# EthanD11/RS-VIO

Hardware: AMD Instinct MI355X
Metric: stereo frames/sec (tracker+BA) on 752×480 EuRoC stream; BA ms/iter at window=10 (higher is better)
Workload: dtype f32 (tracker) / f64 (BA)

## Files before the change

### rs-vio_amd/csrc/ba.hip

```cpp
#include <rccl/rccl.h>

#include <algorithm>
#include <chrono>
#include <cmath>
#include <cstdlib>
#include <cstring>
#include <string>
#include <sys/resource.h>
#include <numeric>
#include <stdexcept>
#include <vector>

#include "common.hpp"

#include "obs_pass.hpp"
#include "se3.hpp"
#include "wave.hpp"

#pragma clang fp contract(fast)

namespace rsvio {

namespace {

// ... 351 lines not shown
            int u = 0;
#pragma unroll
            for (int a = 0; a < 3; ++a) {
#pragma unroll
                for (int c = 0; c < 3; ++c) L.Wr[a * 3 + c] += wt * (J[0][6 + a] * J[0][c] + J[1][6 + a] * J[1][c]);
#pragma unroll
                for (int c = a; c < 3; ++c) L.Ur[u++] += wt * (J[0][6 + a] * J[0][6 + c] + J[1][6 + a] * J[1][6 + c]);
                L.gr[a] += J[0][6 + a] * wr0 + J[1][6 + a] * wr1;
            }
        }
    }
}

__device__ __forceinline__ void wave_sync() {
    __builtin_amdgcn_fence(__ATOMIC_SEQ_CST, "wavefront");
    __builtin_amdgcn_wave_barrier();
}

template <bool WAVE = false>
__device__ void store_linearization(const Work& Wk, int buf, int s, int lane, bool act, bool fr, int first, int nk,
                                    int l, const SlotLin& L, double (*sh)[64]) {
    if (act && fr) {
        double rec[kRawF];
#pragma unroll
        for (int i = 0; i < 6; ++i) rec[RV + i] = L.V[i];
#pragma unroll
        for (int i = 0; i < 3; ++i) rec[RGP + i] = L.gp[i];
#pragma unroll
        for (int i = 0; i < 9; ++i) rec[RWR + i] = L.Wr[i];
#pragma unroll
        for (int i = 0; i < 6; ++i) rec[RUR + i] = L.Ur[i];
#pragma unroll
        for (int i = 0; i < 3; ++i) rec[RGR + i] = L.gr[i];
        rec[27] = 0.0;
        double2* dst = reinterpret_cast<double2*>(Wk.raws[buf] + (size_t)s * kRawF);
#pragma unroll
        for (int i = 0; i < kRawF / 2; ++i) dst[i] = make_double2(rec[2 * i], rec[2 * i + 1]);
    }
#pragma unroll
    for (int i = 0; i < 6; ++i) sh[i][lane] = L.V[i];
#pragma unroll
    for (int i = 0; i < 3; ++i) sh[6 + i][lane] = L.gp[i];
    if constexpr (WAVE) wave_sync(); else __syncthreads();
    if (act && lane == first) {
        double Vl[6] = {0, 0, 0, 0, 0, 0}, gl[3] = {0, 0, 0};
        for (int k = 0; k < nk; ++k) {
#pragma unroll
            for (int i = 0; i < 6; ++i) Vl[i] += sh[i][first + k];
#pragma unroll
            for (int i = 0; i < 3; ++i) gl[i] += sh[6 + i][first + k];
        }
        double rec[kLmF] = {Vl[0], Vl[1], Vl[2], Vl[3], Vl[4], Vl[5], gl[0], gl[1], gl[2], 0.0, 0.0, 0.0};
        double2* dst = reinterpret_cast<double2*>(Wk.rawl[buf] + (size_t)l * kLmF);
#pragma unroll
        for (int i = 0; i < kLmF / 2; ++i) dst[i] = make_double2(rec[2 * i], rec[2 * i + 1]);
    }
}

__device__ __forceinline__ bool chol_inv3(const double A[3][3], double X[3][3]) {
    const double d0 = A[0][0];
    if (!(d0 > 0.0) || !isfinite(d0)) return false;
    const double l00 = sqrt(d0), l10 = A[1][0] / l00, l20 = A[2][0] / l00;
    const double d1 = A[1][1] - l10 * l10;
    if (!(d1 > 0.0) || !isfinite(d1)) return false;
    const double l11 = sqrt(d1), l21 = (A[2][1] - l20 * l10) / l11;
    const double d2 = (A[2][2] - l20 * l20) - l21 * l21;
    if (!(d2 > 0.0) || !isfinite(d2)) return false;
    const double l22 = sqrt(d2);
    const double m00 = 1.0 / l00, m11 = 1.0 / l11, m22 = 1.0 / l22;
    const double m10 = -(l10 * m00) * m11, m21 = -(l21 * m11) * m22;
    const double m20 = -(l20 * m00 + l21 * m10) * m22;
    X[0][0] = (m00 * m00 + m10 * m10) + m20 * m20;
    X[0][1] = X[1][0] = m10 * m11 + m20 * m21;
    X[0][2] = X[2][0] = m20 * m22;
    X[1][1] = m11 * m11 + m21 * m21;
    X[1][2] = X[2][1] = m21 * m22;
    X[2][2] = m22 * m22;
    return true;
}

__device__ __forceinline__ bool landmark_inverse(const double* Vp, double lambda, double Vi[3][3], int chol) {
    double A[3][3] = {{Vp[0] + lambda, Vp[1], Vp[2]}, {Vp[1], Vp[3] + lambda, Vp[4]}, {Vp[2], Vp[4], Vp[5] + lambda}};
    const bool ok = chol ? chol_inv3(A, Vi) : inv3(A, Vi);
    if (!ok)
#pragma unroll
        for (int a = 0; a < 3; ++a)
#pragma unroll
            for (int c = 0; c < 3; ++c) Vi[a][c] = 0.0;
    return ok;
}

struct SlotSrc {
    const unsigned long long* mask;
    const int* lm_base;
    const int* wave_fill;
    const int* wave_lm;
    const unsigned* key;
    const double2* uv;
    int nb_lm, nb_pad;
    int uv32;
};
constexpr unsigned long long kEvenBits = 0x5555555555555555ull;

__device__ void build_slots_body(const Geometry& G, const Prob& Pr, const SlotSrc& S, int4* hdr, double2* huv,
                                 int b) {
    const int t = threadIdx.x;
    const double2 z2 = make_double2(0.0, 0.0);
    if (b < S.nb_lm) {
        const int l = 256 * b + t;
        if (l >= G.n_lm) return;
        const int base = S.lm_base[l];
        if (base < 0) return;
        const unsigned long long m = S.mask[l];
        unsigned long long kb = (m | (m >> 1)) & kEvenBits;
        const int ns = __popcll(kb);
        for (size_t ps = (size_t)base; kb; kb &= kb - 1, ++ps) {
            const int k = (__ffsll((long long)kb) - 1) >> 1;
            const int c0 = (int)(m >> (2 * k)) & 1, c1 = (int)(m >> (2 * k + 1)) & 1;
            const int no = c0 + c1;
            hdr[2 * ps] = make_int4(k, l, base & 63, ns);
            hdr[2 * ps + 1] = make_int4(Pr.free_idx[k], no, no == 2 ? 2 : c1, 0);
            if (no == 1) huv[2 * ps + 1] = z2;
        }
    } else if (b < S.nb_lm + S.nb_pad) {
        const int ps = 256 * (b - S.nb_lm) + t;
        if (ps >= 64 * G.n_wave || (ps & 63) < S.wave_fill[ps >> 6]) return;
        hdr[2 * (size_t)ps] = make_int4(0, 0, 0, 0);
        hdr[2 * (size_t)ps + 1] = make_int4(-1, 0, 0, 0);
        huv[2 * (size_t)ps] = z2;
        huv[2 * (size_t)ps + 1] = z2;
    } else {
        const int i = 256 * (b - S.nb_lm - S.nb_pad) + t;
        if (i >= G.n_obs) return;
        const unsigned key = S.key[i];
        const int l = (int)(key >> 6), k = (int)(key >> 1) & 31, c = (int)(key & 1);
        const unsigned long long m = S.mask[l];
        const unsigned long long below = ((m | (m >> 1)) & kEvenBits) & ((1ull << (2 * k)) - 1ull);
        const size_t q = (size_t)S.lm_base[l] + __popcll(below);
        const int sub = (c == 1 && ((m >> (2 * k)) & 1)) ? 1 : 0;
        if (S.uv32) {
            const float2 f = reinterpret_cast<const float2*>(S.uv)[i];
            huv[2 * q + sub] = make_double2((double)f.x, (double)f.y);
        } else {
            huv[2 * q + sub] = S.uv[i];
        }
    }
}

constexpr int kPairU = 8;

__device__ void build_pairs_body(const Geometry& G, const Prob& Pr, const SlotSrc& S, int4* pairs, int c) {
    __shared__ int cnt[4];
    const int pb = c / kGrp, x = c % kGrp;
    const int fa = Pr.pb_fa[pb], fb = Pr.pb_fb[pb];
    int kfa = 0, kfb = 0;
    for (int k = 0; k < G.n_kf; ++k) {
        const int f = Pr.free_idx[k];
        if (f == fa) kfa = k;
        if (f == fb) kfb = k;
    }
    const unsigned long long ma = 3ull << (2 * kfa), mb = 3ull << (2 * kfb);
    const unsigned long long below_a = (1ull << (2 * kfa)) - 1ull, below_b = (1ull << (2 * kfb)) - 1ull;
    const int tid = threadIdx.x, lane = tid & 63, wave = tid >> 6;
    const int nw = G.n_wave > x ? (G.n_wave - x + kGrp - 1) / kGrp : 0;
    const int k0 = nw * wave / 4, k1 = nw * (wave + 1) / 4;
    int4* out = pairs + (size_t)c * G.pair_stride;
    struct Round {
        int l0[kPairU], l1[kPairU], lbs[kPairU];
        unsigned long long m[kPairU];
    };
    auto load = [&](int kb, Round& R) {
#pragma unroll
        for (int u = 0; u < kPairU; ++u) {
            const int w = x + kGrp * (kb + u);
            const bool in = kb + u < k1;
            R.l0[u] = in ? S.wave_lm[w] : 0;
            R.l1[u] = in ? S.wave_lm[w + 1] : 0;
        }
#pragma unroll
        for (int u = 0; u < kPairU; ++u) {
            const bool in = R.l0[u] + lane < R.l1[u];
            R.m[u] = in ? S.mask[R.l0[u] + lane] : 0ull;
            R.lbs[u] = in ? S.lm_base[R.l0[u] + lane] : 0;
        }
    };
    auto scan = [&](const Round& R, bool write, int& acc) {
#pragma unroll
        for (int u = 0; u < kPairU; ++u) {
            for (int l = R.l0[u] + lane; l - lane < R.l1[u]; l += 64) {
                const bool first = l == R.l0[u] + lane;
                const unsigned long long mm = first ? R.m[u] : (l < R.l1[u] ? S.mask[l] : 0ull);
                const bool has = (mm & ma) && (mm & mb);
                const unsigned long long bal = __ballot(has);
                if (write && has) {
                    const unsigned long long kbits = (mm | (mm >> 1)) & kEvenBits;
                    const int lb = first ? R.lbs[u] : S.lm_base[l];
                    out[acc + __popcll(bal & ((1ull << lane) - 1ull))] =
                        make_int4(lb + __popcll(kbits & below_a), lb + __popcll(kbits & below_b), l, 0);
                }
                acc += __popcll(bal);
            }
        }
    };
    Round R0;
    load(k0, R0);
    int n = 0;
    scan(R0, false, n);
    for (int kb = k0 + kPairU; kb < k1; kb += kPairU) {
        Round R;
        load(kb, R);
        scan(R, false, n);
    }
    if (lane == 0) cnt[wave] = n;
    __syncthreads();
    int base = 0;
    for (int v = 0; v < wave; ++v) base += cnt[v];
    const int total = cnt[0] + cnt[1] + cnt[2] + cnt[3];
    scan(R0, true, base);
    for (int kb = k0 + kPairU; kb < k1; kb += kPairU) {
        Round R;
        load(kb, R);
        scan(R, true, base);
    }
    for (int i = total + tid; i < G.pair_stride; i += 256) out[i] = make_int4(-1, 0, 0, 0);
}

__global__ __launch_bounds__(256) void ba_stage_in(const uint4* src, uint4* __restrict__ dst, int n_words) {
    const int t = (int)(blockIdx.x * 256 + threadIdx.x), st = (int)(gridDim.x * 256);
    const int i0 = t, i1 = t + st;
    uint4 a, b;
    host_load2x16(src + min(i0, n_words - 1), src + min(i1, n_words - 1), a, b);
    if (i0 < n_words) dst[i0] = a;
    if (i1 < n_words) dst[i1] = b;
}

__global__ __launch_bounds__(256) void ba_build_layout(Geometry G, Prob Pr, SlotSrc S, int nb_slots, int4* hdr,
                                                       double2* huv, int4* pairs) {
    const int b = blockIdx.x;
    if (b < nb_slots)
        build_slots_body(G, Pr, S, hdr, huv, b);
    else
        build_pairs_body(G, Pr, S, pairs, b - nb_slots);
}

__device__ void linearize_body(const Geometry& G, const Prob& Pr, const Work& Wk, int w, int with_reset,
                               double lambda0) {
    __shared__ double sh[10][64];
    const int lane = threadIdx.x;
    const int s = 64 * w + lane;
    if (with_reset) {
        const int nt = G.n_wave * 64;
        for (int i = s; i < 7 * G.n_kf; i += nt) {
            Wk.pose[0][i] = Wk.pose_init[i];
            Wk.pose[1][i] = Wk.pose_init[i];
        }
        for (int i = s; i < 3 * G.n_lm; i += nt) {
            Wk.pw[0][i] = Wk.pw_init[i];
            Wk.pw[1][i] = Wk.pw_init[i];
        }
        if (s == 0) {
            Wk.tick[1] = wall_clock64();
            *Wk.singular = 0;
            LmState st{};
            st.lambda = lambda0;
            st.nu = 2.0;
            *Wk.st = st;
        }
    }
    const double* pose0 = with_reset ? Wk.pose_init : Wk.pose[0];
    const double* pw0 = with_reset ? Wk.pw_init : Wk.pw[0];
    const int4 h0 = Pr.slot_hdr[2 * s], h1 = Pr.slot_hdr[2 * s + 1];
    const double2 uvq[2] = {Pr.slot_uv[2 * s], Pr.slot_uv[2 * s + 1]};
    STAMP(11);
    const bool act = h1.y > 0;
    const int kf = h0.x, l = h0.y, first = act ? h0.z : lane, nk = act ? h0.w : 1;
    const bool fr = h1.x >= 0;
    SlotLin L;
    if (act) {
        const Pose P = pose_from7(pose0 + 7 * kf);
        const double* pwp = pw0 + 3 * l;
        const double p[3] = {pwp[0], pwp[1], pwp[2]};
        slot_linearize(G, P, p, h1.y, h1.z, uvq, fr, L);
    } else {
        const Pose P{};
        const double p[3] = {0.0, 0.0, 1.0};
        slot_linearize(G, P, p, 0, 0, uvq, false, L);
    }
    STAMP(12);
    store_linearization(Wk, 0, s, lane, act, fr, first, nk, l, L, sh);
    const double c = wave_sum_det(L.cost);
    if (lane == 0) {
        Wk.partA[w * kPartA] = c;
        Wk.partA[w * kPartA + 1] = 0.0;
    }
    STAMP(14);
}

__global__ __launch_bounds__(64) void ba_linearize(Geometry G, Prob Pr, Work Wk, double lambda0) {
    linearize_body(G, Pr, Wk, blockIdx.x, 1, lambda0);
}

__device__ void trial_scalars_wave(const Geometry& G, const Prob& Pr, const Work& Wk, const LmState& s,
                                   int include_poses, double out[4]) {
    const int lane = threadIdx.x & 63;
    constexpr int kU = 8;
    double4 pv[kU];
    const int wl = max(G.n_wave - 1, 0), el = 7 * G.n_kf - 1;
#pragma unroll
    for (int k = 0; k < kU; ++k)
        pv[k] = *reinterpret_cast<const double4*>(Wk.partD + (size_t)min(lane + 64 * k, wl) * kPartD);
    double p0[3], p1[3];
    int fi[3];
#pragma unroll
    for (int k = 0; k < 3; ++k) {
        const int e = min(lane + 64 * k, el);
        fi[k] = Pr.free_idx[e / 7];
        p0[k] = Wk.pose[0][e];
        p1[k] = Wk.pose[1][e];
    }
#pragma unroll
    for (int k = 0; k < kU; ++k)
        if (lane + 64 * k >= G.n_wave) pv[k] = make_double4(0.0, 0.0, 0.0, 0.0);
    bool fr[3];
#pragma unroll
    for (int k = 0; k < 3; ++k) fr[k] = include_poses && lane + 64 * k <= el && fi[k] >= 0;
    double acc[kPartD] = {0.0, 0.0, 0.0, 0.0};
#pragma unroll
    for (int k = 0; k < kU; ++k) {
        acc[0] += pv[k].x;
        acc[1] += pv[k].y;
        acc[2] += pv[k].z;
        acc[3] += pv[k].w;
    }
    for (int i = lane + 64 * kU; i < G.n_wave; i += 64) {
        const double4 v = *reinterpret_cast<const double4*>(Wk.partD + (size_t)i * kPartD);
        acc[0] += v.x;
        acc[1] += v.y;
        acc[2] += v.z;
        acc[3] += v.w;
    }
    double sq[2] = {0.0, 0.0};
#pragma unroll
    for (int k = 0; k < 3; ++k)
        if (fr[k]) {
            sq[0] += p0[k] * p0[k];
            sq[1] += p1[k] * p1[k];
        }
    if (!s.solve_ok)
#pragma unroll
        for (int k = 0; k < kPartD; ++k) acc[k] = 0.0;
    acc[3] += sq[s.cur];
#pragma unroll
    for (int k = 0; k < kPartD; ++k) out[k] = wave_sum_det(acc[k]);
}

__device__ void trial_scalars_p2p(const Geometry& G, const Prob& Pr, const Work& Wk, const LmState& s, const P2P& P,
                                  unsigned long long gen, int* err, double out[4]) {
    const int lane = threadIdx.x & 63, par = (int)(gen & 1);
    double* own = P.peer[P.rank];
    const int el = 7 * G.n_kf - 1;
    double p0[3], p1[3];
    int fi[3];
#pragma unroll
    for (int k = 0; k < 3; ++k) {
        const int e = min(lane + 64 * k, el);
        fi[k] = Pr.free_idx[e / 7];
        p0[k] = Wk.pose[0][e];
        p1[k] = Wk.pose[1][e];
    }
    double sq[2] = {0.0, 0.0};
#pragma unroll
    for (int k = 0; k < 3; ++k)
        if (lane + 64 * k <= el && fi[k] >= 0) {
            sq[0] += p0[k] * p0[k];
            sq[1] += p1[k] * p1[k];
        }
    for (int j = 0; j < 4; ++j) out[j] = 0.0;
    bool late = false;
    for (int r = 0; r < P.nranks; ++r) {
        const int nw = P.xnw[r];
        double acc[kPartD] = {0.0, 0.0, 0.0, 0.0};
        for (int w = lane; w < max(nw, 512); w += 64) {
            double4 v = make_double4(0.0, 0.0, 0.0, 0.0);
            if (w < nw) {
                const unsigned long long* f = p2p_tflag(own, par, r, w);
                long long spins = 0;
                while (__hip_atomic_load(f, __ATOMIC_RELAXED, __HIP_MEMORY_SCOPE_SYSTEM) < gen) {
                    __builtin_amdgcn_s_sleep(1);
                    if (++spins > (1ll << 25)) {
                        late = true;
                        break;
                    }
                }
                __builtin_amdgcn_fence(__ATOMIC_ACQUIRE, "");
                const double* q = p2p_tval(own, par, r, w);
// ... 2205 lines not shown
    for (int k = 1; k < kPartD; ++k) mv = i == k ? out[k] : mv;
    double got = mv;
    if (r < nr && r != me) {
        ll_put(p2p_ll(P.peer[r], par, me) + 2 * i, mv, g32);
        const unsigned long long* w = p2p_ll(P.peer[me], par, r) + 2 * i;
        long long spins = 0;
        for (;;) {
            const unsigned long long a = __hip_atomic_load(w, __ATOMIC_RELAXED, __HIP_MEMORY_SCOPE_SYSTEM);
            const unsigned long long b = __hip_atomic_load(w + 1, __ATOMIC_RELAXED, __HIP_MEMORY_SCOPE_SYSTEM);
            if ((unsigned)(a >> 32) == g32 && (unsigned)(b >> 32) == g32) {
                got = __longlong_as_double((long long)((a & 0xffffffffull) | (b << 32)));
                break;
            }
            if (++spins > (1ll << 25)) {
                late = true;
                got = 0.0;
                break;
            }
            __builtin_amdgcn_s_sleep(1);
        }
    }
    if (late) atomicExch(err, 1);
    double v4[kPartD];
#pragma unroll
    for (int k = 0; k < kPartD; ++k) {
        double v = 0.0;
        for (int q = 0; q < nr; ++q) v += rl64(got, 4 * q + k);
        v4[k] = v;
    }
    if (lane == 0) {
#pragma unroll
        for (int k = 0; k < kPartD; ++k) Wk.trial4[k] = v4[k];
        *xgen = gen;
    }
}

__global__ __launch_bounds__(64) void ba_backsub_relinearize_p2p3(Geometry G, Prob Pr, Work Wk, P2P P,
                                                                  unsigned long long* xgen, int* err,
                                                                  unsigned long long* k6tag) {
    __shared__ double sh[10][64];
    __shared__ double shp[3][64];
    __shared__ double shs[4][64];
    if ((int)blockIdx.x == G.n_wave) {
        if (G.n_wave <= 256)
            k6_reduce_p2p<4>(G, Pr, Wk, P, xgen, err, k6tag);
        else
            k6_reduce_p2p<8>(G, Pr, Wk, P, xgen, err, k6tag);
        return;
    }
    unsigned long long gen = *xgen + 1;
    __asm__ volatile("" : "+s"(gen));
    k6_body<false>(G, Pr, Wk, blockIdx.x, threadIdx.x, sh, shp, shs, nullptr, gen, k6tag);
}

__device__ void k6_last_push(const Geometry& G, const Prob& Pr, const Work& Wk, const P2P& P,
                             unsigned long long* xgen, unsigned long long gen, const unsigned long long* k6part,
                             const LmState& s) {
    const int lane = threadIdx.x & 63;
    constexpr int kU = 8;
    const int wl = max(G.n_wave - 1, 0), el = 7 * G.n_kf - 1;
    unsigned long long pw[kU][kPartD];
#pragma unroll
    for (int k = 0; k < kU; ++k)
#pragma unroll
        for (int j = 0; j < kPartD; ++j)
            pw[k][j] = __hip_atomic_load(k6part + (size_t)min(lane + 64 * k, wl) * kPartD + j, __ATOMIC_RELAXED,
                                         __HIP_MEMORY_SCOPE_AGENT);
    double p0[3], p1[3];
    int fi[3];
#pragma unroll
    for (int k = 0; k < 3; ++k) {
        const int e = min(lane + 64 * k, el);
        fi[k] = Pr.free_idx[e / 7];
        p0[k] = Wk.pose[0][e];
        p1[k] = Wk.pose[1][e];
    }
    double acc[kPartD] = {0.0, 0.0, 0.0, 0.0};
#pragma unroll
    for (int k = 0; k < kU; ++k)
#pragma unroll
        for (int j = 0; j < kPartD; ++j)
            acc[j] += lane + 64 * k < G.n_wave ? __longlong_as_double((long long)pw[k][j]) : 0.0;
    for (int i = lane + 64 * kU; i < G.n_wave; i += 64)
#pragma unroll
        for (int j = 0; j < kPartD; ++j)
            acc[j] += __longlong_as_double((long long)__hip_atomic_load(k6part + (size_t)i * kPartD + j, __ATOMIC_RELAXED,
                                                                        __HIP_MEMORY_SCOPE_AGENT));
    double sq[2] = {0.0, 0.0};
#pragma unroll
    for (int k = 0; k < 3; ++k)
        if (P.rank == 0 && lane + 64 * k <= el && fi[k] >= 0) {
            sq[0] += p0[k] * p0[k];
            sq[1] += p1[k] * p1[k];
        }
    acc[3] += sq[s.cur];
    double out[kPartD];
#pragma unroll
    for (int k = 0; k < kPartD; ++k) out[k] = wave_sum_det(acc[k]);
    const int r = lane >> 2, i = lane & 3, par = (int)(gen & 1);
    double mv = out[0];
#pragma unroll
    for (int k = 1; k < kPartD; ++k) mv = i == k ? out[k] : mv;
    if (r < P.nranks) ll_put(p2p_ll(P.peer[r], par, P.rank) + 2 * i, mv, (unsigned)gen);
    if (lane == 0) *xgen = gen;
}

__global__ __launch_bounds__(64) void ba_backsub_relinearize_p2p4(Geometry G, Prob Pr, Work Wk, P2P P,
                                                                  unsigned long long* xgen, unsigned* k6cnt,
                                                                  unsigned long long* k6part) {
    __shared__ double sh[10][64];
    __shared__ double shp[3][64];
    __shared__ double shs[4][64];
    unsigned long long gen = *xgen + 1;
    __asm__ volatile("" : "+s"(gen));
    if (G.n_wave > 0) {
        k6_body<false>(G, Pr, Wk, blockIdx.x, threadIdx.x, sh, shp, shs, nullptr, gen, nullptr, k6part);
        const LmState s = *Wk.st;
        if (s.done || !s.solve_ok) return;
        __builtin_amdgcn_s_waitcnt(kWaitStores);
        __builtin_amdgcn_fence(__ATOMIC_RELEASE, "agent");
        unsigned t = 0;
        if (threadIdx.x == 0) t = __hip_atomic_fetch_add(k6cnt, 1u, __ATOMIC_ACQ_REL, __HIP_MEMORY_SCOPE_AGENT);
        t = __builtin_amdgcn_readfirstlane(t);
        if (t != (unsigned)G.n_wave - 1) return;
        __builtin_amdgcn_fence(__ATOMIC_ACQUIRE, "agent");
        if (threadIdx.x == 0) __hip_atomic_store(k6cnt, 0u, __ATOMIC_RELAXED, __HIP_MEMORY_SCOPE_AGENT);
        k6_last_push(G, Pr, Wk, P, xgen, gen, k6part, s);
    } else {
        const LmState s = *Wk.st;
        if (s.done || !s.solve_ok) return;
        k6_last_push(G, Pr, Wk, P, xgen, gen, k6part, s);
    }
}

__global__ __launch_bounds__(64) void ba_reduce_trial(Geometry G, Prob Pr, Work Wk, int include_poses) {
    const LmState s = *Wk.st;
    if (s.done) return;
    double v[4];
    trial_scalars_wave(G, Pr, Wk, s, include_poses, v);
    if (threadIdx.x == 0)
        for (int k = 0; k < 4; ++k) Wk.trial4[k] = v[k];
}

constexpr int kK7Threads = 256;
#ifndef RSVIO_K7_BLOCKS
#define RSVIO_K7_BLOCKS 16
#endif
constexpr int kK7Blocks = RSVIO_K7_BLOCKS;
__device__ __forceinline__ void lm_decide_body(const Geometry& G, const Prob& Pr, const Work& Wk, int pre_reduced,
                                               const LmArgs& la, LmState* host, unsigned long long* htick,
                                               double* hout, const P2P* PP = nullptr,
                                               const unsigned long long* xgen = nullptr, int* err = nullptr) {
    STAMP(8);
    __shared__ LmState sd;
    if (threadIdx.x < 64) {
        const LmState d = lm_decide(G, Pr, Wk, Wk.st_prev, pre_reduced, la, PP, xgen, err);
        if (threadIdx.x == 0) {
            sd = d;
            if (blockIdx.x == 0) {
                LmState h = d;
                h.p2p_err = Wk.p2p_err ? *Wk.p2p_err : 0;
                *Wk.st = d;
                *host = h;
            }
        }
    }
    __syncthreads();
    const LmState s = sd;
    if (hout && s.done) {
        const double* pose = Wk.pose[s.cur];
        const double* pw = Wk.pw[s.cur];
        const int np = 7 * G.n_kf, n = np + 3 * G.n_lm;
        const int per = (((n + (int)gridDim.x - 1) / (int)gridDim.x) + 1) & ~1;
        const int i0 = (int)blockIdx.x * per, i1 = min(n, i0 + per);
        for (int i = i0 + 2 * (int)threadIdx.x; i < i1; i += 2 * kK7Threads) {
            const double a = i < np ? pose[i] : pw[i - np];
            if (i + 1 < i1) {
                const double b = i + 1 < np ? pose[i + 1] : pw[i + 1 - np];
                *reinterpret_cast<double2*>(hout + i) = make_double2(a, b);
            } else {
                hout[i] = a;
            }
        }
        __threadfence_system();
        __syncthreads();
        if (threadIdx.x == 0)
            __hip_atomic_store(htick + 4 + blockIdx.x, Wk.tick[1], __ATOMIC_RELEASE, __HIP_MEMORY_SCOPE_SYSTEM);
    }
    if (blockIdx.x == 0 && threadIdx.x == 0) {
        const unsigned long long t = Wk.tick[0] + 1;
        Wk.tick[0] = t;
        htick[1] = Wk.tick[1];
        htick[2] = wall_clock64();
        __threadfence_system();
        __hip_atomic_store(htick, t, __ATOMIC_RELEASE, __HIP_MEMORY_SCOPE_SYSTEM);
    }
    STAMP(10);
}

__global__ __launch_bounds__(kK7Threads) void ba_lm_decide(Geometry G, Prob Pr, Work Wk, int pre_reduced, LmArgs la,
                                                           LmState* host, unsigned long long* htick, double* hout) {
    lm_decide_body(G, Pr, Wk, pre_reduced, la, host, htick, hout);
}

__global__ __launch_bounds__(kK7Threads) void ba_lm_decide_p2p(Geometry G, Prob Pr, Work Wk, LmArgs la, LmState* host,
                                                               unsigned long long* htick, double* hout, P2P P,
                                                               const unsigned long long* xgen, int* err, int mode) {
    lm_decide_body(G, Pr, Wk, mode, la, host, htick, hout, &P, xgen, err);
}

struct WinDesc {
    Geometry G;
    Prob Pr;
    Work W[4];
    int skip;
};

__device__ __forceinline__ void desc_touch1(const void* p) { __asm__ volatile("" ::"s"(p)); }
template <class... T>
__device__ __forceinline__ void desc_touch(const T*... p) {
    (desc_touch1(p), ...);
}


__global__ __launch_bounds__(64) void bab_linearize(const WinDesc* __restrict__ D, double lambda0) {
    const WinDesc& d = D[blockIdx.y];
    const int skip = d.skip, bound = d.G.n_wave;
    const Prob Pr = d.Pr;
    const Work& Wk = d.W[2];
    desc_touch(Pr.slot_hdr, Pr.slot_uv, Wk.pose_init, Wk.pw_init, Wk.st);
    if (skip | ((int)blockIdx.x >= bound)) return;
    linearize_body(d.G, Pr, Wk, blockIdx.x, 1, lambda0);
}

__global__ __launch_bounds__(kSchurThreads) void bab_schur_chunks(const WinDesc* __restrict__ D, int wi, LmArgs la) {
    const WinDesc& d = D[blockIdx.y];
    const int skip = d.skip, bound = d.G.n_chunk;
    const Prob Pr = d.Pr;
    const Work& Wk = d.W[wi];
    desc_touch(Pr.pairs, Wk.partD, Wk.pose[0], Wk.pose[1], Wk.st_prev, Wk.st);
    if (skip | ((int)blockIdx.x >= bound)) return;
    schur_chunks_body(d.G, Pr, Wk, la, 0, blockIdx.x);
}

template <int NF>
__global__ __launch_bounds__(kK5Threads) void bab_camera_solve(const WinDesc* __restrict__ D, int wi) {
    const WinDesc& d = D[blockIdx.x];
    const int skip = d.skip, nkf = d.G.n_kf, nf = d.G.n_free, npb = d.G.n_pb, nw = d.G.n_wave;
    const Prob Pr = d.Pr;
    const Work& Wk = d.W[wi];
    desc_touch(Pr.free_idx, Pr.dmap, Wk.pose[0], Wk.pose[1], Wk.cpart, Wk.partA, Wk.singular, Wk.st);
    __asm__ volatile("" ::"s"(nkf), "s"(nf), "s"(npb), "s"(nw));
    if (skip) return;
    camera_solve_mfma_body<NF>(d.G, Pr, Wk, 1);
}

template <int NF>
__global__ __launch_bounds__(64 * kBkWaves) void bab_camera_solve_blk(const WinDesc* __restrict__ D, int wi) {
    const WinDesc& d = D[blockIdx.x];
    const int skip = d.skip;
    const Prob Pr = d.Pr;
    const Work& Wk = d.W[wi];
    desc_touch(Pr.free_idx, Pr.dmap, Wk.pose[0], Wk.pose[1], Wk.cpart, Wk.partA, Wk.singular, Wk.st);
    if (skip) return;
    camera_solve_blk_body<NF>(d.G, Pr, Wk, 1);
}

__global__ __launch_bounds__(64) void bab_backsub_relinearize(const WinDesc* __restrict__ D, int wi) {
    const WinDesc& d = D[blockIdx.y];
    const int skip = d.skip, bound = d.G.n_wave;
    const Prob Pr = d.Pr;
    const Work& Wk = d.W[wi];
    desc_touch(Pr.slot_hdr, Pr.slot_uv, Wk.st, Wk.raws[0], Wk.raws[1], Wk.rawl[0], Wk.rawl[1], Wk.pw[0], Wk.pw[1],
               Wk.pose[0], Wk.pose[1], Wk.dc);
    if (skip | ((int)blockIdx.x >= bound)) return;
    __shared__ double sh[10][64];
    __shared__ double shp[3][64];
    __shared__ double shs[4][64];
    k6_body<false>(d.G, Pr, Wk, blockIdx.x, threadIdx.x, sh, shp, shs);
}

__global__ __launch_bounds__(kK7Threads) void bad_lm_decide(const WinDesc* __restrict__ D, int wi, LmArgs la,
                                                            LmState* host, unsigned long long* htick, double* hout) {
    const WinDesc& d = D[0];
    const Prob Pr = d.Pr;
    const Work& Wk = d.W[wi];
    lm_decide_body(d.G, Pr, Wk, 0, la, host, htick, hout);
}

__global__ __launch_bounds__(64) void bab_lm_decide(const WinDesc* __restrict__ D, int wi, LmArgs la, LmState* host) {
    const WinDesc& d = D[blockIdx.x];
    if (d.skip) return;
    const LmState s = lm_decide(d.G, d.Pr, d.W[wi], d.W[wi].st, 0, la);
    if (threadIdx.x == 0) {
        *d.W[wi].st = s;
        host[blockIdx.x] = s;
    }
}


__device__ void p2p_exchange(const double* msg, int n, const P2P& P, unsigned long long* xgen, int* err, double* out,
                             unsigned long long gen_pre = 0) {
    __shared__ unsigned long long sgen;
    const int tid = threadIdx.x, nr = P.nranks, me = P.rank;
    if (!gen_pre) {
        if (tid == 0) sgen = *xgen + 1;
        __syncthreads();
    }
    const unsigned long long gen = gen_pre ? gen_pre : sgen;
    const int par = (int)(gen & 1);
    if (n <= kP2PLLMax) {
        const unsigned g32 = (unsigned)gen;
        const int r = tid / kP2PLLMax, i = tid % kP2PLLMax;
        if (r < nr && i < n) ll_put(p2p_ll(P.peer[r], par, me) + 2 * i, msg[i], g32);
        __shared__ double got[kP2PMax][kP2PLLMax];
        if (r < nr && i < n) {
            const unsigned long long* w = p2p_ll(P.peer[me], par, r) + 2 * i;
            long long spins = 0;
            for (;;) {
                const unsigned long long a = __hip_atomic_load(w, __ATOMIC_RELAXED, __HIP_MEMORY_SCOPE_SYSTEM);
                const unsigned long long b = __hip_atomic_load(w + 1, __ATOMIC_RELAXED, __HIP_MEMORY_SCOPE_SYSTEM);
                if ((unsigned)(a >> 32) == g32 && (unsigned)(b >> 32) == g32) {
                    got[r][i] = __longlong_as_double((long long)((a & 0xffffffffull) | (b << 32)));
                    break;
                }
                if (++spins > (1ll << 25)) {
                    atomicExch(err, 1);
                    got[r][i] = 0.0;
                    break;
                }
                __builtin_amdgcn_s_sleep(1);
            }
        }
        __syncthreads();
        if (tid < n) {
            double v = 0.0;
            for (int q = 0; q < nr; ++q) v += got[q][tid];
            out[tid] = v;
        }
        if (tid == 0) *xgen = gen;
        return;
    }
    for (int r = 0; r < nr; ++r) {
        double* dst = P.peer[r] + (size_t)(par * kP2PMax + me) * kP2PMsg;
        for (int i = tid; i < n; i += 256) dst[i] = msg[i];
    }
    __threadfence_system();
    __syncthreads();
    if (tid < nr)
// ... 46 lines not shown
    combine_system<256>(G, Pr, Wk, msg, st->lambda, P.rank == 0);
    __syncthreads();
    if (threadIdx.x == 0) *Wk.singular = 0;
    p2p_exchange(msg, (int)sys_len(G), P, xgen, err, Wk.sys);
}

__global__ __launch_bounds__(256) void ba_p2p_trial(Geometry G, Prob Pr, Work Wk, P2P P, unsigned long long* xgen,
                                                    int* err) {
    __shared__ double msg[4];
    const unsigned long long gen = *xgen + 1;
    const LmState s = *Wk.st;
    if (s.done) return;
    if (threadIdx.x < 64) {
        double v[4];
        trial_scalars_wave(G, Pr, Wk, s, P.rank == 0 ? 1 : 0, v);
        if (threadIdx.x == 0)
            for (int k = 0; k < 4; ++k) msg[k] = v[k];
    }
    __syncthreads();
    p2p_exchange(msg, 4, P, xgen, err, Wk.trial4, gen);
}

}

RSVIO_DBG_READER(rsvio_dbg_ba_stamps)
RSVIO_RT_READER(rsvio_dbg_ba_rt)

using rsvio_obs::observation_pass;

__attribute__((target("popcnt"))) static inline int slot_count(unsigned long long m) {
    return __builtin_popcountll((m | (m >> 1)) & kEvenBits);
}

struct BundleAdjuster {
    rsvio_ba_params P{};
    hipStream_t stream = nullptr;
    bool own_stream = true;
    hipEvent_t ev0 = nullptr, ev1 = nullptr;
    Geometry G{};
    bool has_problem = false;
    int iter_chunk = 2;
    struct GraphSlot {
        hipGraphExec_t exec = nullptr;
        int k = -1;
        rsvio_lm_cfg cfg{};
        bool exp = false, stale = false;
        int nf = -1, coll = -1, wcap = 0, chunk = -1;
        const void* dptr = nullptr;
        hipEvent_t ev_launch = nullptr;
    };
    GraphSlot gv, gd;
    int solves_of_problem = 0;
    bool graphs_ok = true;
    int k5_variant = 2;
    std::vector<hipGraphExec_t> retired;
    void drop_slot(GraphSlot& sl) {
        if (sl.exec) {
            if (!settled) {
                if (hipStreamQuery(stream) == hipSuccess)
                    settled = true;
                else
                    (void)hipGetLastError();
            }
            if (settled) {
                destroy_retired();
                (void)hipGraphExecDestroy(sl.exec);
            } else {
                retired.push_back(sl.exec);
                if (retired.size() > 4) settle();
            }
        }
        sl.exec = nullptr;
        sl.k = -1;
        sl.stale = false;
    }
    void drop_graph() {
        drop_slot(gv);
        drop_slot(gd);
    }
    void destroy_retired() {
        for (hipGraphExec_t g : retired) (void)hipGraphExecDestroy(g);
        retired.clear();
    }
    static bool same_cfg(const rsvio_lm_cfg& a, const rsvio_lm_cfg& b) {
        return a.max_iterations == b.max_iterations && a.cost_tolerance == b.cost_tolerance &&
               a.parameter_tolerance == b.parameter_tolerance && a.huber_delta == b.huber_delta &&
               a.lambda_init == b.lambda_init && a.linear_solver == b.linear_solver;
    }
    bool graph_update = true;
    bool desc_on = true;
    WinDesc hdesc{};
    double desc_huber = std::nan("");
    int desc_chol = -1;
    HostBuf<WinDesc> h_desc1;
    hipEvent_t ev_desc = nullptr;
    bool desc_pending = false;
    bool desc_mode() const { return desc_on && coll == 0 && k5_variant == 2 && G.n_free <= 10 && G.n_wave > 0; }
    int fold_lvl = 3;
    int fold_req = 3;
    bool p2p_shared_gpu = false;
    bool p2p_fold() const { return fold_lvl >= 1 && coll == 2 && k5_variant == 2 && G.n_free <= 10; }
    bool p2p_fold2() const { return fold_lvl == 2 && p2p_fold(); }
    bool p2p_fold3() const { return fold_lvl == 3 && p2p_fold() && k6_fits(); }
    int k6_cap = 0;
    bool k6_fits() const { return G.n_wave + 1 <= k6_cap; }
    int p2p_share = 1;
    bool p2p_fold4() const { return fold_lvl == 4 && p2p_fold(); }
    const WinDesc* dptr() const { return reinterpret_cast<const WinDesc*>(d_arena.p + lay.desc); }
    void fill_desc(WinDesc& d) const {
        d = WinDesc{};
        d.G = G;
        d.G.huber_delta = desc_huber;
        d.G.chol = desc_chol;
        d.Pr = prob();
        d.W[0] = work(0);
        d.W[1] = work(1);
        d.W[2] = work_at(0);
        d.W[3] = work_at(1);
        d.skip = 0;
    }
    void refresh_desc() {
        if (desc_pending && hipEventQuery(ev_desc) != hipSuccess) {
            (void)hipGetLastError();
            RSVIO_HIP(hipEventSynchronize(ev_desc));
        }
        desc_pending = false;
        desc_huber = G.huber_delta;
        desc_chol = G.chol;
        hdesc.G.huber_delta = desc_huber;
        hdesc.G.chol = desc_chol;
        if (!h_desc1.p) h_desc1.alloc(1);
        *h_desc1.p = hdesc;
        settled = false;
        RSVIO_HIP(hipMemcpyAsync(d_arena.p + lay.desc, h_desc1.p, sizeof(WinDesc), hipMemcpyHostToDevice, stream));
        RSVIO_HIP(hipEventRecord(ev_desc, stream));
        desc_pending = true;
    }
    bool start_graph(const rsvio_lm_cfg& cfg, int& k) {
        if (coll == 1 || !graphs_ok) return false;
        const bool dm = desc_mode() && solves_of_problem == 0;
        ++solves_of_problem;
        GraphSlot& sl = dm ? gd : gv;
        if (dm && (G.huber_delta != desc_huber || G.chol != desc_chol)) refresh_desc();
        const int wcap = (G.n_wave + G.n_wave / 4 + kGrp - 1) / kGrp * kGrp;
        const bool k_ok = sl.k == k || (dm && sl.k > k && sl.k <= k + 2);
        const bool topo = sl.exec && k_ok && same_cfg(sl.cfg, cfg) && sl.exp == export_on && sl.nf == G.n_free &&
                          sl.coll == coll;
        const bool hit = topo && (dm ? (sl.dptr == dptr() && sl.chunk == G.n_chunk && G.n_wave <= sl.wcap &&
                                        2 * G.n_wave > sl.wcap)
                                     : !sl.stale);
        if (hit) k = sl.k;
        if (!hit) {
            const auto tg0 = std::chrono::steady_clock::now();
            bool try_update = topo && sl.k == k && graph_update;
            if (try_update && hipEventQuery(sl.ev_launch) != hipSuccess) {
                (void)hipGetLastError();
                try_update = false;
            }
            if (!try_update) drop_slot(sl);
            if (hipStreamBeginCapture(stream, hipStreamCaptureModeThreadLocal) != hipSuccess) {
                (void)hipGetLastError();
                graphs_ok = false;
                return false;
            }
            bool ok = true;
            try {
                if (dm) {
                    enqueue_start_d(cfg.lambda_init, wcap);
                    for (int i = 0; i < k; ++i) enqueue_iteration_d(cfg, i, wcap);
                    enqueue_decide_d(cfg, k);
                } else {
                    enqueue_start(cfg.lambda_init);
                    for (int i = 0; i < k; ++i) enqueue_iteration(cfg, i);
                    enqueue_decide(cfg, k);
                }
            } catch (...) {
                ok = false;
            }
            hipGraph_t g = nullptr;
            if (hipStreamEndCapture(stream, &g) != hipSuccess) ok = false;
            const auto tg1 = std::chrono::steady_clock::now();
            bool updated = false;
            if (ok && try_update) {
                hipGraphNode_t err_node = nullptr;
                hipGraphExecUpdateResult r = hipGraphExecUpdateError;
                updated = hipGraphExecUpdate(sl.exec, g, &err_node, &r) == hipSuccess && r == hipGraphExecUpdateSuccess;
                if (!updated) {
                    (void)hipGetLastError();
                    drop_slot(sl);
                }
            }
            if (ok && !updated && hipGraphInstantiate(&sl.exec, g, nullptr, nullptr, 0) != hipSuccess) {
                sl.exec = nullptr;
                ok = false;
            }
            const auto tg2 = std::chrono::steady_clock::now();
            if (g) (void)hipGraphDestroy(g);
            if (prof_env)
                fprintf(stderr, "[rsvio] graph us (%s): drop+capture %.1f %s %.1f destroy %.1f\n", dm ? "desc" : "value",
                        std::chrono::duration<double, std::micro>(tg1 - tg0).count(),
                        updated ? "update" : "instantiate",
                        std::chrono::duration<double, std::micro>(tg2 - tg1).count(),
                        std::chrono::duration<double, std::micro>(std::chrono::steady_clock::now() - tg2).count());
            if (!ok) {
                (void)hipGetLastError();
                graphs_ok = false;
                return false;
            }
            sl.k = k;
            sl.cfg = cfg;
            sl.exp = export_on;
            sl.nf = G.n_free;
            sl.coll = coll;
            sl.stale = false;
            sl.wcap = wcap;
            sl.chunk = G.n_chunk;
            sl.dptr = dm ? static_cast<const void*>(dptr()) : nullptr;
        }
        settled = false;
        RSVIO_HIP(hipGraphLaunch(sl.exec, stream));
        if (graph_update) RSVIO_HIP(hipEventRecord(sl.ev_launch, stream));
        return true;
    }
    int last_iterations = 3;
    DevBuf<double> d_pose2, d_pw2;
    DevBuf<uint8_t> d_arena;
    HostBuf<uint8_t> h_arena;
    bool up_pending = false;
    struct ArenaLayout {
        size_t desc, pose_init, pw_init, free_idx, pb_fa, pb_fb, dmap, mask, lm_base, wave_fill, wave_lm, key, ouv, upload;
        size_t hdr, uv, pairs, total;
    } lay{};
    bool prof_env = false;
    bool prof_slow = false;
    std::string prof_maps;
    bool uv_env = true;
    bool early_env = false;
    bool stage_kernel = true;
    bool stage_split = true;
    const void* h_arena_dev = nullptr;
    HostBuf<double> h_out;
    bool state_export = false, export_on = false;
    bool state_fresh = false;
    std::vector<int> hs_free, hs_pb_fa, hs_pb_fb;
    DevBuf<double> d_raws, d_rawl, d_partA, d_partD, d_cpart, d_sys, d_dc, d_trial4;
    DevBuf<int> d_singular;
    size_t n_pad = 0;
    DevBuf<LmState> d_state;
    HostBuf<LmState> h_state;
    DevBuf<unsigned long long> d_tick;
    unsigned long long* h_tick = nullptr;
    unsigned long long n_tick = 0;
    bool settled = true, tick_wait = true;
    double wclk_khz = 1.0e5;
    ncclComm_t comm = nullptr;
    int nranks = 1, rank = 0;
    int coll = 0;
    bool sharded() const { return coll != 0; }
    double* xbuf = nullptr;
    P2P p2p{};
    bool p2p_opened[kP2PMax] = {};
    DevBuf<int> d_p2p_err;
    DevBuf<unsigned long long> d_xgen;
    DevBuf<int> d_xnw;
    DevBuf<unsigned long long> d_k6tag;
    DevBuf<unsigned> d_k6cnt;

    void init(const rsvio_ba_params& p) {
        P = p;
        if (P.max_keyframes < 2 || P.max_keyframes > kMaxFree + 1 || P.max_landmarks < 1 ||
            P.max_landmarks > (1 << 26) || P.max_observations < 1)
            throw std::invalid_argument("invalid BA capacities (max_keyframes in [2, 21], max_landmarks <= 2^26)");
        RSVIO_HIP(hipSetDevice(P.device));
        RSVIO_HIP(hipStreamCreateWithFlags(&stream, hipStreamNonBlocking));
        RSVIO_HIP(hipEventCreate(&ev0));
        RSVIO_HIP(hipEventCreate(&ev1));
        RSVIO_HIP(hipEventCreateWithFlags(&gv.ev_launch, hipEventDisableTiming));
        RSVIO_HIP(hipEventCreateWithFlags(&gd.ev_launch, hipEventDisableTiming));
        RSVIO_HIP(hipEventCreateWithFlags(&ev_desc, hipEventDisableTiming));
        const char* fv = std::getenv("RSVIO_P2P_FOLD");
        if (fv && fv[0] >= '0' && fv[0] <= '4') fold_lvl = fold_req = fv[0] - '0';
        const char* dv = std::getenv("RSVIO_BA_DESC");
        desc_on = !(dv && dv[0] == '0');
        const char* gu = std::getenv("RSVIO_BA_GRAPH_UPDATE");
        graph_update = !(gu && gu[0] == '0');
        h_state.alloc(1, hipHostMallocCoherent);
        h_out.alloc((size_t)7 * P.max_keyframes + (size_t)3 * P.max_landmarks, hipHostMallocCoherent);
        d_tick.alloc(2);
        RSVIO_HIP(hipMemset(d_tick.p, 0, 2 * sizeof(unsigned long long)));
        RSVIO_HIP(hipHostMalloc(reinterpret_cast<void**>(&h_tick), (4 + kK7Blocks) * sizeof(unsigned long long),
                                hipHostMallocCoherent));
        std::memset(h_tick, 0, (4 + kK7Blocks) * sizeof(unsigned long long));
        {
            int khz = 0;
            if (hipDeviceGetAttribute(&khz, hipDeviceAttributeWallClockRate, P.device) == hipSuccess && khz > 0)
                wclk_khz = khz;
        }
        const char* wv = std::getenv("RSVIO_BA_WAIT");
        tick_wait = !(wv && std::strcmp(wv, "sync") == 0);
        const char* ge = std::getenv("RSVIO_BA_GRAPHS");
        graphs_ok = !(ge && ge[0] == '0');
        const char* pv = std::getenv("RSVIO_BA_PROFILE");
        prof_env = pv != nullptr;
        prof_slow = pv && std::strcmp(pv, "slow") == 0;
        const char* u32v = std::getenv("RSVIO_BA_UV32");
        uv_env = !(u32v && u32v[0] == '0');
        const char* ecv = std::getenv("RSVIO_BA_EARLY_COPY");
        early_env = ecv && ecv[0] == '1';
        const char* stv = std::getenv("RSVIO_BA_STAGE");
        stage_kernel = !(stv && std::strcmp(stv, "sdma") == 0);
        if (stage_kernel) early_env = false;
        const char* ssv = std::getenv("RSVIO_BA_STAGE_SPLIT");
        stage_split = stage_kernel && !(ssv && ssv[0] == '0');
        const char* kv = std::getenv("RSVIO_K5");
        if (kv && std::strcmp(kv, "gj1") == 0) k5_variant = 1;
        if (kv && std::strcmp(kv, "pipe4") == 0) k5_variant = 0;
        if (kv && std::strcmp(kv, "mfma") == 0) k5_variant = 2;
    }
    ~BundleAdjuster() {
        if (stream) (void)hipStreamSynchronize(stream);
        settled = true;
        if (h_tick) (void)hipHostFree(h_tick);
        drop_graph();
        destroy_retired();
        if (comm) ncclCommDestroy(comm);
        for (int r = 0; r < kP2PMax; ++r)
            if (p2p_opened[r]) (void)hipIpcCloseMemHandle(p2p.peer[r]);
        if (xbuf) (void)hipFree(xbuf);
        if (ev0) (void)hipEventDestroy(ev0);
        if (ev1) (void)hipEventDestroy(ev1);
        if (gv.ev_launch) (void)hipEventDestroy(gv.ev_launch);
        if (gd.ev_launch) (void)hipEventDestroy(gd.ev_launch);
        if (ev_desc) (void)hipEventDestroy(ev_desc);
        if (stream && own_stream) (void)hipStreamDestroy(stream);
    }

    template <class T>
    static void grow(DevBuf<T>& b, size_t n) {
        if (b.n < n) b.alloc(std::max<size_t>(n, 1));
    }
    Prob prob() const {
        Prob p;
        p.free_idx = reinterpret_cast<const int*>(d_arena.p + lay.free_idx);
        p.slot_hdr = reinterpret_cast<const int4*>(d_arena.p + lay.hdr);
        p.slot_uv = reinterpret_cast<const double2*>(d_arena.p + lay.uv);
        p.pairs = reinterpret_cast<const int4*>(d_arena.p + lay.pairs);
        p.pb_fa = reinterpret_cast<const int*>(d_arena.p + lay.pb_fa);
        p.pb_fb = reinterpret_cast<const int*>(d_arena.p + lay.pb_fb);
        p.dmap = reinterpret_cast<const int*>(d_arena.p + lay.dmap);
        return p;
    }
    Work work(int it) const {
        Work w = work_at((it + 1) & 1);
        w.st_prev = d_state.p + (it & 1);
        return w;
    }
    Work work_at(int si) const {
        Work w;
        w.pose[0] = d_pose2.p; w.pose[1] = d_pose2.p + 7 * (size_t)G.n_kf;
        w.pw[0] = d_pw2.p; w.pw[1] = d_pw2.p + 3 * (size_t)std::max(G.n_lm, 1);
        w.pose_init = reinterpret_cast<const double*>(d_arena.p + lay.pose_init);
        w.pw_init = reinterpret_cast<const double*>(d_arena.p + lay.pw_init);
        w.raws[0] = d_raws.p; w.raws[1] = d_raws.p + (size_t)kRawF * std::max<size_t>(n_pad, 1);
        w.rawl[0] = d_rawl.p; w.rawl[1] = d_rawl.p + (size_t)kLmF * std::max(G.n_lm, 1);
        w.singular = d_singular.p;
        w.p2p_err = coll == 2 ? d_p2p_err.p : nullptr;
        w.partA = d_partA.p; w.partD = d_partD.p;
        w.cpart = d_cpart.p;
        w.sys = d_sys.p; w.dc = d_dc.p; w.trial4 = d_trial4.p;
        w.st = d_state.p + si;
        w.st_prev = w.st;
        w.tick = d_tick.p;
        return w;
    }
// ... 1287 lines not shown
```

### rs-vio_amd/csrc/common.hpp

```cpp
#pragma once
#include <hip/hip_runtime.h>

#include <cstdint>
#include <cstdio>
#include <stdexcept>
#include <string>

#include "rsvio_gpu.h"

namespace rsvio {

void set_last_error(const std::string& msg);

struct HipError {
    hipError_t err;
    std::string where;
};

#define RSVIO_HIP(expr)                                                                    \
    do {                                                                                   \
        hipError_t _e = (expr);                                                            \
        if (_e != hipSuccess)                                                              \
            throw ::rsvio::HipError{_e, std::string(#expr) + " @ " + __FILE__ + ":" +      \
                                            std::to_string(__LINE__)};                     \
    } while (0)

struct CallOrderError : std::invalid_argument {
    using std::invalid_argument::invalid_argument;
};

template <class F>
int guarded(F&& f) {
    try {
        return f();
    } catch (const HipError& e) {
        set_last_error(std::string("HIP error ") + hipGetErrorString(e.err) + " in " + e.where);
        return RSVIO_ERR_HIP;
    } catch (const std::bad_alloc&) {
        set_last_error("host allocation failed");
        return RSVIO_ERR_NOMEM;
    } catch (const std::invalid_argument& e) {
        set_last_error(e.what());
        return RSVIO_ERR_INVALID_ARG;
    } catch (const std::exception& e) {
        set_last_error(e.what());
        return RSVIO_ERR_INTERNAL;
    }
}

#ifdef RSVIO_STAMPS
#define RSVIO_DBG_DECL static __device__ unsigned long long g_dbg[4096 * 32];
#define STAMP(k)                                                              \
    do {                                                                      \
        if (threadIdx.x == 0 && blockIdx.x < 4096) {                          \
            __builtin_amdgcn_s_waitcnt(0);                                    \
            g_dbg[blockIdx.x * 32 + (k)] = (unsigned long long)clock64();     \
        }                                                                     \
    } while (0)
#define RSVIO_DBG_READER(name)                                                             \
    extern "C" int name(unsigned long long* out, int n) {                                  \
        if (n > 4096 * 32) n = 4096 * 32;                                                  \
        return (int)hipMemcpyFromSymbol(out, HIP_SYMBOL(g_dbg), sizeof(unsigned long long) * n); \
    }
#define RSVIO_RT_DECL static __device__ unsigned long long g_rt[4096 * 16];
#define RTSTAMP(k)                                                                              \
    do {                                                                                        \
        if (threadIdx.x == 0 && blockIdx.x < 4096)                                              \
            g_rt[blockIdx.x * 16 + (k)] = (unsigned long long)__builtin_amdgcn_s_memrealtime();  \
    } while (0)
#define RSVIO_RT_READER(name)                                                              \
    extern "C" int name(unsigned long long* out, int n) {                                  \
        if (n > 4096 * 16) n = 4096 * 16;                                                  \
        return (int)hipMemcpyFromSymbol(out, HIP_SYMBOL(g_rt), sizeof(unsigned long long) * n); \
    }
#else
#define RSVIO_RT_DECL
#define RTSTAMP(k) \
    do {           \
    } while (0)
#define RSVIO_RT_READER(name)
#define RSVIO_DBG_DECL
#define STAMP(k) \
    do {         \
    } while (0)
#define RSVIO_DBG_READER(name)
#endif

struct TrackerView {
    hipStream_t stream;
    const rsvio_feature* out[2];
    const float2* undist[2];
    int n[2];
    int device;
};
TrackerView tracker_view(rsvio_tracker* t);

__device__ __forceinline__ uint32_t sat_u32(float v) {
    const uint32_t t = (uint32_t)fminf(fmaxf(v, 0.0f), 4294967040.0f);
    return v >= 4294967296.0f ? 0xFFFFFFFFu : (v > 0.0f ? t : 0u);
}

__device__ __forceinline__ void host_load2x16(const void* a, const void* b, uint4& va, uint4& vb) {
    __asm__ volatile(
        "global_load_dwordx4 %0, %2, off sc0 sc1\n\t"
        "global_load_dwordx4 %1, %3, off sc0 sc1\n\t"
        "s_waitcnt vmcnt(0)"
        : "=&v"(va), "=&v"(vb)
        : "v"(a), "v"(b)
        : "memory");
}

__host__ __device__ inline uint32_t level_w(uint32_t w, int i) { return w / (1u << i); }
__host__ __device__ inline uint32_t level_h(uint32_t h, int i) { return h / (1u << i); }
__host__ __device__ inline size_t level_offset(uint32_t w, uint32_t h, int level) {
    size_t off = 0;
    for (int i = 0; i < level; ++i) off += (size_t)level_w(w, i) * level_h(h, i);
    return off;
}

template <class T>
struct DevBuf {
    T* p = nullptr;
    size_t n = 0;
    DevBuf() = default;
    explicit DevBuf(size_t count) { alloc(count); }
    void alloc(size_t count) {
        release();
        if (count) RSVIO_HIP(hipMalloc(&p, count * sizeof(T)));
        n = count;
    }
    void release() {
        if (p) (void)hipFree(p);
        p = nullptr;
        n = 0;
    }
    ~DevBuf() { release(); }
    DevBuf(const DevBuf&) = delete;
    DevBuf& operator=(const DevBuf&) = delete;
};

template <class T>
struct HostBuf {
    T* p = nullptr;
    size_t n = 0;
    void alloc(size_t count, unsigned flags = hipHostMallocDefault) {
        release();
        if (count) RSVIO_HIP(hipHostMalloc(&p, count * sizeof(T), flags));
        n = count;
    }
    void release() {
        if (p) (void)hipHostFree(p);
        p = nullptr;
        n = 0;
    }
    ~HostBuf() { release(); }
};

}
```

Before: 5000.

## Prefetch LM export values before decide, ballot keyframe lookup, add realtime stamps

In the LM decide kernel, threads outside the first wave now load both candidate pose and landmark buffers into registers before lm_decide runs. Once the decision is known, the first chunk of the host export is written from those registers instead of reloading after the barrier, which hides global load latency behind the decide step. In build_pairs, the serial loop searching for the keyframe index is replaced with a wave ballot and find-first-set. The change also adds row-indexed realtime timing stamps that compile away unless debugging is on, and disables graph update and event recording when dm is set. The cost is double the export loads, and the first wave no longer takes part in the export loop.

```diff
diff --git a/rs-vio_amd/csrc/ba.hip b/rs-vio_amd/csrc/ba.hip
--- a/rs-vio_amd/csrc/ba.hip
+++ b/rs-vio_amd/csrc/ba.hip
@@ -527,16 +527,10 @@
 __device__ void build_pairs_body(const Geometry& G, const Prob& Pr, const SlotSrc& S, int4* pairs, int c) {
     __shared__ int cnt[4];
     const int pb = c / kGrp, x = c % kGrp;
+    const int tid = threadIdx.x, lane = tid & 63, wave = tid >> 6;
+    const int fk = lane < G.n_kf ? Pr.free_idx[lane] : -2;
     const int fa = Pr.pb_fa[pb], fb = Pr.pb_fb[pb];
-    int kfa = 0, kfb = 0;
-    for (int k = 0; k < G.n_kf; ++k) {
-        const int f = Pr.free_idx[k];
-        if (f == fa) kfa = k;
-        if (f == fb) kfb = k;
-    }
-    const unsigned long long ma = 3ull << (2 * kfa), mb = 3ull << (2 * kfb);
-    const unsigned long long below_a = (1ull << (2 * kfa)) - 1ull, below_b = (1ull << (2 * kfb)) - 1ull;
-    const int tid = threadIdx.x, lane = tid & 63, wave = tid >> 6;
+    unsigned long long ma, mb, below_a, below_b;
     const int nw = G.n_wave > x ? (G.n_wave - x + kGrp - 1) / kGrp : 0;
     const int k0 = nw * wave / 4, k1 = nw * (wave + 1) / 4;
     int4* out = pairs + (size_t)c * G.pair_stride;
@@ -579,6 +573,12 @@
     };
     Round R0;
     load(k0, R0);
+    {
+        const unsigned long long ba = __ballot(fk == fa), bb = __ballot(fk == fb);
+        const int kfa = ba ? __ffsll((long long)ba) - 1 : 0, kfb = bb ? __ffsll((long long)bb) - 1 : 0;
+        ma = 3ull << (2 * kfa), mb = 3ull << (2 * kfb);
+        below_a = (1ull << (2 * kfa)) - 1ull, below_b = (1ull << (2 * kfb)) - 1ull;
+    }
     int n = 0;
     scan(R0, false, n);
     for (int kb = k0 + kPairU; kb < k1; kb += kPairU) {
@@ -612,10 +612,16 @@
 __global__ __launch_bounds__(256) void ba_build_layout(Geometry G, Prob Pr, SlotSrc S, int nb_slots, int4* hdr,
                                                        double2* huv, int4* pairs) {
     const int b = blockIdx.x;
+    RTSTAMP_ROW(b, 12);
     if (b < nb_slots)
         build_slots_body(G, Pr, S, hdr, huv, b);
     else
         build_pairs_body(G, Pr, S, pairs, b - nb_slots);
+    RTSTAMP_SYNC();
+    if (b < nb_slots)
+        RTSTAMP_ROW(b, 10);
+    else
+        RTSTAMP_ROW(b - nb_slots, 11);
 }
 
 __device__ void linearize_body(const Geometry& G, const Prob& Pr, const Work& Wk, int w, int with_reset,
@@ -3127,6 +3133,24 @@
                                                double* hout, const P2P* PP = nullptr,
                                                const unsigned long long* xgen = nullptr, int* err = nullptr) {
     STAMP(8);
+    RTSTAMP_ROW(4080 + blockIdx.x, 12);
+    constexpr int kExport = kK7Threads - 64;
+    const int np = 7 * G.n_kf, n = np + 3 * G.n_lm;
+    const int per = (((n + (int)gridDim.x - 1) / (int)gridDim.x) + 1) & ~1;
+    const int i0 = (int)blockIdx.x * per, i1 = min(n, i0 + per);
+    const int et = (int)threadIdx.x - 64;
+    const int ef = i0 + 2 * et;
+    double e0[2] = {0.0, 0.0}, e1[2] = {0.0, 0.0};
+    if (hout && et >= 0) {
+#pragma unroll
+        for (int k = 0; k < 2; ++k) {
+            const int e = min(ef + k, n - 1);
+            const bool in_pose = e < np;
+            const int o = in_pose ? e : e - np;
+            e0[k] = (in_pose ? Wk.pose[0] : Wk.pw[0])[o];
+            e1[k] = (in_pose ? Wk.pose[1] : Wk.pw[1])[o];
+        }
+    }
     __shared__ LmState sd;
     if (threadIdx.x < 64) {
         const LmState d = lm_decide(G, Pr, Wk, Wk.st_prev, pre_reduced, la, PP, xgen, err);
@@ -3142,19 +3166,27 @@
     }
     __syncthreads();
     const LmState s = sd;
+    RTSTAMP_ROW(blockIdx.x, 13);
     if (hout && s.done) {
-        const double* pose = Wk.pose[s.cur];
-        const double* pw = Wk.pw[s.cur];
-        const int np = 7 * G.n_kf, n = np + 3 * G.n_lm;
-        const int per = (((n + (int)gridDim.x - 1) / (int)gridDim.x) + 1) & ~1;
-        const int i0 = (int)blockIdx.x * per, i1 = min(n, i0 + per);
-        for (int i = i0 + 2 * (int)threadIdx.x; i < i1; i += 2 * kK7Threads) {
-            const double a = i < np ? pose[i] : pw[i - np];
-            if (i + 1 < i1) {
-                const double b = i + 1 < np ? pose[i + 1] : pw[i + 1 - np];
-                *reinterpret_cast<double2*>(hout + i) = make_double2(a, b);
-            } else {
-                hout[i] = a;
+        if (et >= 0) {
+            if (ef < i1) {
+                const double a = s.cur ? e1[0] : e0[0], b = s.cur ? e1[1] : e0[1];
+                RTSTAMP_ROW_T(64, blockIdx.x, 14);
+                if (ef + 1 < i1)
+                    *reinterpret_cast<double2*>(hout + ef) = make_double2(a, b);
+                else
+                    hout[ef] = a;
+            }
+            const double* pose = Wk.pose[s.cur];
+            const double* pw = Wk.pw[s.cur];
+            for (int i = ef + 2 * kExport; i < i1; i += 2 * kExport) {
+                const double a = i < np ? pose[i] : pw[i - np];
+                if (i + 1 < i1) {
+                    const double b = i + 1 < np ? pose[i + 1] : pw[i + 1 - np];
+                    *reinterpret_cast<double2*>(hout + i) = make_double2(a, b);
+                } else {
+                    hout[i] = a;
+                }
             }
         }
         __threadfence_system();
@@ -3170,6 +3202,7 @@
         __threadfence_system();
         __hip_atomic_store(htick, t, __ATOMIC_RELEASE, __HIP_MEMORY_SCOPE_SYSTEM);
     }
+    RTSTAMP_ROW(blockIdx.x, 15);
     STAMP(10);
 }
 
@@ -3522,7 +3555,7 @@
         if (hit) k = sl.k;
         if (!hit) {
             const auto tg0 = std::chrono::steady_clock::now();
-            bool try_update = topo && sl.k == k && graph_update;
+            bool try_update = !dm && topo && sl.k == k && graph_update;
             if (try_update && hipEventQuery(sl.ev_launch) != hipSuccess) {
                 (void)hipGetLastError();
                 try_update = false;
@@ -3589,7 +3622,7 @@
         }
         settled = false;
         RSVIO_HIP(hipGraphLaunch(sl.exec, stream));
-        if (graph_update) RSVIO_HIP(hipEventRecord(sl.ev_launch, stream));
+        if (graph_update && !dm) RSVIO_HIP(hipEventRecord(sl.ev_launch, stream));
         return true;
     }
     int last_iterations = 3;
diff --git a/rs-vio_amd/csrc/common.hpp b/rs-vio_amd/csrc/common.hpp
--- a/rs-vio_amd/csrc/common.hpp
+++ b/rs-vio_amd/csrc/common.hpp
@@ -68,6 +68,15 @@
         if (threadIdx.x == 0 && blockIdx.x < 4096)                                              \
             g_rt[blockIdx.x * 16 + (k)] = (unsigned long long)__builtin_amdgcn_s_memrealtime();  \
     } while (0)
+#define RTSTAMP_ROW(row, k) RTSTAMP_ROW_T(0, row, k)
+#define RTSTAMP_ROW_T(t, row, k)                                                                \
+    do {                                                                                        \
+        if (threadIdx.x == (t) && (unsigned)(row) < 4096u) {                                    \
+            __builtin_amdgcn_s_waitcnt(0);                                                      \
+            g_rt[(row) * 16 + (k)] = (unsigned long long)__builtin_amdgcn_s_memrealtime();       \
+        }                                                                                       \
+    } while (0)
+#define RTSTAMP_SYNC() __syncthreads()
 #define RSVIO_RT_READER(name)                                                              \
     extern "C" int name(unsigned long long* out, int n) {                                  \
         if (n > 4096 * 16) n = 4096 * 16;                                                  \
@@ -77,6 +86,15 @@
 #define RSVIO_RT_DECL
 #define RTSTAMP(k) \
     do {           \
+    } while (0)
+#define RTSTAMP_ROW(row, k) \
+    do {                    \
+    } while (0)
+#define RTSTAMP_ROW_T(t, row, k) \
+    do {                         \
+    } while (0)
+#define RTSTAMP_SYNC() \
+    do {               \
     } while (0)
 #define RSVIO_RT_READER(name)
 #define RSVIO_DBG_DECL
```

New measurement: 4916. 0.983x the previous value.
